# bluenote-1577/floria

Measured on AMD Instinct MI355X. Metric: SNP-blocks phased/sec (whole node), higher is better.
Workload: dtype u64 (Q24 fixed-point allele weights) + f64 scores

## Files before the change

### floria_amd/csrc/floria_hip.hip

```cpp
#include <hip/hip_runtime.h>

#include <algorithm>
#include <cmath>
#include <cstdint>
#include <cstdio>
#include <cstdlib>
#include <cstring>
#include <limits>
#include <numeric>
#include <string>
#include <utility>
#include <atomic>
#include <chrono>
#include <mutex>
#include <thread>
#include <type_traits>
#include <vector>

#include "../../include/floria_hip.h"
#include "beam_kernel.h"
#include "wave_util.h"
#include "beam_slab_kernel.h"
#include "beam_wide_kernel.h"
#include "optimize_kernel.h"
#include "reassign_kernel.h"
#include "hapq_kernel.h"
#include "blocks_kernel.h"
#include "graph_kernel.h"
#include "stats_kernel.h"
#include "realign_kernel.h"
#include "realign_walk_kernel.h"
#include "pileup_kernel.h"
#include "realign_gather_kernel.h"
#include "upload_kernel.h"
#include "assemble_kernel.h"
#include "assemble_order_kernel.h"
#include "mono_kernel.h"
#include "span_kernel.h"

static_assert(FLORIA_MAX_PLOIDY == fl::MAX_PLOIDY, "ploidy limits out of sync");

namespace {

thread_local std::string g_err;
int fail(int code, const std::string& msg) { g_err = msg; return code; }

#define HIPCHK(expr)                                                                                   \
    do {                                                                                               \
        hipError_t _e = (expr);                                                                        \
        if (_e != hipSuccess)                                                                          \
            return fail(_e == hipErrorOutOfMemory ? FLORIA_E_NOMEM : FLORIA_E_DEVICE,                  \
                        std::string(#expr) + ": " + hipGetErrorString(_e));                            \
    } while (0)

constexpr double DIV_FACTOR  = 0.25;
constexpr double PROB_CUTOFF = 0.01;
constexpr uint32_t BINOM_NMAX_CAP = 1024;

struct DevBuf {
    void* p = nullptr;
    size_t cap = 0;
    int ensure(size_t bytes) {
        if (bytes <= cap) return 0;
        if (p) { (void)hipFree(p); p = nullptr; cap = 0; }
        size_t want = bytes + bytes / 8 + 256;
        hipError_t e = hipMalloc(&p, want);
        if (e != hipSuccess) { p = nullptr; return fail(FLORIA_E_NOMEM, std::string("hipMalloc(") + std::to_string(want) + "): " + hipGetErrorString(e)); }
        cap = want;
        return 0;
    }
    void release() { if (p) (void)hipFree(p); p = nullptr; cap = 0; }
    template <class T> T* as() const { return (T*)p; }
};

struct Seg { size_t off, bytes; };
struct Carve {
    size_t cursor = 0;
    char* base = nullptr;
    Seg seg(size_t bytes) { const Seg s{cursor, bytes}; cursor += (bytes + 255) & ~(size_t)255; return s; }
    int place(DevBuf& buf) { const int rc = buf.ensure(cursor + 256); base = buf.as<char>(); return rc; }
    template <class T = void> T* at(Seg s) const { return (T*)(base + s.off); }
    hipError_t up(Seg s, const void* src, size_t bytes, hipStream_t st) const { return bytes ? hipMemcpyAsync(base + s.off, src, bytes, hipMemcpyHostToDevice, st) : hipSuccess; }
};

struct HostBox {
    char* h = nullptr;
    char* d = nullptr;
    size_t cap = 0;
    int ensure(size_t bytes) {
        if (bytes <= cap) return 0;
        release();
        const size_t want = bytes + bytes / 4 + 4096;
        hipError_t e = hipHostMalloc((void**)&h, want, hipHostMallocMapped);
        if (e == hipSuccess) e = hipHostGetDevicePointer((void**)&d, h, 0);
        if (e != hipSuccess) { if (h) (void)hipHostFree(h); h = nullptr; d = nullptr; return fail(FLORIA_E_NOMEM, std::string("hipHostMalloc(mapped, ") + std::to_string(want) + "): " + hipGetErrorString(e)); }
        cap = want;
        return 0;
    }
    void release() { if (h) (void)hipHostFree(h); h = nullptr; d = nullptr; cap = 0; }
};

struct StagePool {
    static constexpr size_t SEG = 16u << 20;
    static constexpr uint32_t NBUF = 8;
    char* buf[NBUF] = {};
    hipEvent_t ev[NBUF] = {};
    bool used[NBUF] = {};
    int init() {
        for (uint32_t i = 0; i < NBUF; ++i) if (!buf[i]) {
            if (hipHostMalloc((void**)&buf[i], SEG, hipHostMallocDefault) != hipSuccess) return fail(FLORIA_E_NOMEM, "hipHostMalloc(staging) failed");
            if (hipEventCreateWithFlags(&ev[i], hipEventDisableTiming) != hipSuccess) return fail(FLORIA_E_DEVICE, "hipEventCreate failed");
        }
        return 0;
    }
    void release() { for (uint32_t i = 0; i < NBUF; ++i) { if (buf[i]) (void)hipHostFree(buf[i]); if (ev[i]) (void)hipEventDestroy(ev[i]); buf[i] = nullptr; ev[i] = nullptr; used[i] = false; } }
};

uint64_t splitmix64(uint64_t& s) {
    uint64_t z = (s += 0x9e3779b97f4a7c15ull);
    z = (z ^ (z >> 30)) * 0xbf58476d1ce4e5b9ull;
    z = (z ^ (z >> 27)) * 0x94d049bb133111ebull;
    return z ^ (z >> 31);
}

}

namespace {
struct BigCache {
    std::mutex m;
    std::vector<std::pair<void*, size_t>> v;
    void* get(size_t n) {
        {
            std::lock_guard<std::mutex> l(m);
            for (size_t i = 0; i < v.size(); ++i)
                if (v[i].second >= n && v[i].second <= 2 * n + 4096) { void* b = v[i].first; v.erase(v.begin() + i); return (char*)b + 64; }
        }
        void* b = malloc(n + 64);
        if (!b) return nullptr;
        *(size_t*)b = n;
        return (char*)b + 64;
    }
    void put(void* payload) {
        if (!payload) return;
        void* b = (char*)payload - 64;
        const size_t cap = *(size_t*)b;
        std::lock_guard<std::mutex> l(m);
        if (cap >= (1u << 20) && v.size() < 8) v.push_back({b, cap}); else free(b);
    }
};
BigCache g_big;
}

struct Knobs {
    uint32_t groups = 0;
    uint32_t beam_path = 0;
    uint32_t no_specialized = 0;
    uint32_t no_p1_shortcut = 0;
    uint32_t opt_threads = 0;
    uint32_t opt_global = 0;
    int32_t  speculate = -1;
    uint32_t upload_chunks = 0;
    uint32_t trace = 0;
    uint32_t spec_gate_div = 2;
    uint32_t reassign_path = 0;
    uint32_t no_bulk = 0;
    uint32_t fx_tags = 0;
    uint32_t arith_ow6 = 0;
    uint32_t asm_order_general = 0;
    uint32_t chain_wgs = 0;
    uint32_t arith_replay = 0;
    uint32_t arith_hbm = 0;
    uint32_t opt_block_order = 0;
    uint32_t s2_assign_only = 0;
    uint32_t arith = 0;
    int32_t  tail_overlap = 0;
    uint32_t tail_waves = 2;
};

struct Arena;

struct floria_hip_ctx {
    int device = 0;
    uint32_t hw_queues = 0;
    hipStream_t stream = nullptr;
    uint32_t user_slots = 0;
    Knobs knobs;
    int n_cu = 256;
    static constexpr uint32_t MAX_GROUPS = 8;
    static constexpr uint32_t MAX_LANES = 32;
    hipStream_t gstream[MAX_LANES] = {};
    hipStream_t gstream_low[MAX_LANES] = {};
    hipEvent_t ev_fork[MAX_LANES] = {}, ev_join[MAX_LANES] = {};
    hipEvent_t ev_gate[MAX_GROUPS] = {};
    hipStream_t tstream[MAX_GROUPS] = {};
    hipEvent_t ev_tail[MAX_GROUPS] = {}, ev_tail_join[MAX_GROUPS] = {};
    hipStream_t copy_stream = nullptr;
    hipEvent_t ev_rids = nullptr;
    hipEvent_t ev_chunk[MAX_GROUPS + 1] = {};
    hipEvent_t ev_copied[MAX_GROUPS + 1] = {};
    hipStream_t flat_stream = nullptr;
    HostBox box;
    double binom_eps = -1.0;
    uint32_t binom_nmax = 0;
    DevBuf d_binom;
    DevBuf d_hash;
    uint32_t hash_len = 0;
    uint32_t w24[256];
    DevBuf d_w24;
    uint64_t Rk1[FLORIA_MAX_PLOIDY], Rk2[FLORIA_MAX_PLOIDY];
    DevBuf state_pool, hist_pool, opt_hist, opt_dist, opt_gain, opt_key, opt_moves, misc, misc0;
    uint32_t cur_len_max = 0;
    uint64_t upload_epoch = 0, ord_epoch = ~0ull, ord_sig = 0;
    const uint2* cur_ord = nullptr; const uint64_t* cur_ord_off = nullptr;
    DevBuf arith_ord, arith_scr, arith_tab, arith_pool;
    floria_timing timing{};
    uint64_t batch_token = 0, token_counter = 0;
    fl::BlockSet last_bs{};
    const uint8_t* last_part = nullptr;
    const uint32_t* last_best = nullptr;
    uint32_t last_nall = 2;
    std::vector<uint32_t> last_bc, last_start, last_end;
    DevBuf graph_buf, graph_hist, graph_sort;
    DevBuf up_tmp;
    std::vector<Arena*> arena_cache;
    StagePool stage;
    DevBuf pile_in, pile_out;
    uint64_t res_token = 0;
    const floria_record_summary* res_summary = nullptr;
    uint32_t res_n_contigs = 0;
    std::vector<uint32_t> res_contig;
    const uint64_t* res_cell_off = nullptr; const uint32_t* res_snp = nullptr; const uint8_t *res_allele = nullptr, *res_qual = nullptr;
    const uint32_t* res_seq_pos = nullptr;
    DevBuf asm_plan;
// ... 1410 lines not shown
                          if (P > 3) { stages.emplace_back(); for (uint32_t p = 4; p <= P; ++p) stages.back().push_back(p); } }
    else for (uint32_t p = 1; p <= P; ++p) stages.push_back({p});
    if (spec == 3 && P < 5) { stages.clear(); for (uint32_t p = 1; p <= P; ++p) stages.push_back({p}); }
    return stages;
}

int s1_core(floria_hip_ctx* ctx, const S1Contigs& SC, const uint32_t* blk_contig, const uint32_t* blk_start, const uint32_t* blk_end,
            uint32_t n_blocks, const floria_params* prm, floria_block_result** out) {
    const uint32_t n_contigs = (uint32_t)SC.cdev.size();
    const Trace TR(ctx->knobs.trace);
    TR.mark("s1_core enter");
    if (prm->max_ploidy < 1 || prm->max_ploidy > FLORIA_MAX_PLOIDY) return fail(FLORIA_E_INVALID, "max_ploidy must be in 1..16");
    if (prm->beam < 1) return fail(FLORIA_E_INVALID, "beam (max_number_solns) must be >= 1");
    if (!(prm->epsilon > 0.0 && prm->epsilon < 1.0)) return fail(FLORIA_E_INVALID, "epsilon must be in (0,1)");
    ctx->timing = floria_timing{};
    ctx->batch_token = 0;
    const uint32_t P = prm->max_ploidy;

    std::vector<uint32_t> bc(n_blocks, 0);
    uint32_t n_max = 1, span_max = 1;
    const uint32_t len_max = SC.len_max, nall = SC.nall;
    const bool any_q0 = SC.any_q0;
    for (uint32_t b = 0; b < n_blocks; ++b) {
        const uint32_t ci = blk_contig ? blk_contig[b] : 0;
        if (ci >= n_contigs) return fail(FLORIA_E_INVALID, "blk_contig out of range");
        bc[b] = ci;
    }
    const std::vector<fl::ContigDev>& cdev = SC.cdev;
    Carve C0;
    const Seg s_cdev = C0.seg(sizeof(fl::ContigDev) * std::max(1u, n_contigs)), s_bc = C0.seg(4ull * n_blocks + 4), s_bs = C0.seg(4ull * n_blocks + 4),
              s_be = C0.seg(4ull * n_blocks + 4), s_p0 = C0.seg(4ull * n_blocks + 4), s_sp = C0.seg(4ull * n_blocks + 4), s_cnt = C0.seg(4ull * n_blocks + 4),
              s_bytes = C0.seg(8ull * n_blocks + 8), s_roff = C0.seg(8ull * (n_blocks + 1));
    int rc = C0.place(ctx->misc0); if (rc) return rc;
    EventTimer T(ctx->stream);
    static_assert(sizeof(fl::ContigDev) % 4 == 0, "box_copy_kernel moves 4-byte words");
    size_t box_cur = 0;
    auto box_take = [&](size_t bytes) { const size_t o = box_cur; box_cur += (bytes + 63) & ~(size_t)63; return o; };
    const size_t bx_cdev = box_take(sizeof(fl::ContigDev) * n_contigs), bx_bc = box_take(4ull * n_blocks), bx_bs = box_take(4ull * n_blocks), bx_be = box_take(4ull * n_blocks),
                 bx_cnt = box_take(4ull * n_blocks), bx_span = box_take(4ull * n_blocks), bx_bytes = box_take(8ull * n_blocks), bx_roff = box_take(8ull * (n_blocks + 1)),
                 bx_jobs = box_take(4ull * n_blocks);
    rc = ctx->box.ensure(box_cur + 64); if (rc) return rc;
    auto box_up = [&](void* dst, const void* src, size_t bytes, size_t at) -> hipError_t {
        if (!bytes) return hipSuccess;
        memcpy(ctx->box.h + at, src, bytes);
        const uint32_t words = (uint32_t)(bytes / 4);
        hipLaunchKernelGGL(box_copy_kernel, dim3(std::max(1u, std::min(256u, (words + 255) / 256))), dim3(256), 0, ctx->stream, (uint32_t*)dst, (const uint32_t*)(ctx->box.d + at), words);
        return hipGetLastError();
    };
    int th = T.begin(K_H2D);
    HIPCHK(box_up(C0.at(s_cdev), cdev.data(), sizeof(fl::ContigDev) * n_contigs, bx_cdev));
    if (n_blocks) {
        HIPCHK(box_up(C0.at(s_bc), bc.data(), 4ull * n_blocks, bx_bc));
        HIPCHK(box_up(C0.at(s_bs), blk_start, 4ull * n_blocks, bx_bs));
        HIPCHK(box_up(C0.at(s_be), blk_end, 4ull * n_blocks, bx_be));
    }
    T.end(th);
    fl::ScanArgs sa{};
    sa.contigs = C0.at<const fl::ContigDev>(s_cdev);
    sa.blk_contig = C0.at<const uint32_t>(s_bc); sa.blk_start = C0.at<const uint32_t>(s_bs); sa.blk_end = C0.at<const uint32_t>(s_be);
    sa.n_blocks = n_blocks; sa.max_ploidy = P;
    sa.cnt = C0.at<uint32_t>(s_cnt); sa.pos0 = C0.at<uint32_t>(s_p0); sa.span = C0.at<uint32_t>(s_sp); sa.bytes = C0.at<uint64_t>(s_bytes);
    sa.h_cnt = (uint32_t*)(ctx->box.d + bx_cnt); sa.h_span = (uint32_t*)(ctx->box.d + bx_span); sa.h_bytes = (uint64_t*)(ctx->box.d + bx_bytes);
    std::vector<uint32_t> cnt(n_blocks, 0), span(n_blocks, 0);
    std::vector<uint64_t> blk_bytes(n_blocks, 0), roff(n_blocks + 1, 0);
    if (n_blocks) {
        int tk = T.begin(K_SEL);
        hipLaunchKernelGGL(fl::block_reads_kernel<false>, dim3(n_blocks), dim3(64), 0, ctx->stream, sa);
        T.end(tk);
        HIPCHK(hipGetLastError());
        HIPCHK(hipStreamSynchronize(ctx->stream));
        memcpy(cnt.data(), ctx->box.h + bx_cnt, 4ull * n_blocks);
        memcpy(span.data(), ctx->box.h + bx_span, 4ull * n_blocks);
        memcpy(blk_bytes.data(), ctx->box.h + bx_bytes, 8ull * n_blocks);
    }
    TR.mark("block counts on the host");
    uint64_t algo_bytes = 0;
    for (uint32_t b = 0; b < n_blocks; ++b) {
        roff[b + 1] = roff[b] + cnt[b];
        n_max = std::max(n_max, cnt[b]); span_max = std::max(span_max, span[b]);
        algo_bytes += blk_bytes[b];
    }
    if (n_max >= (1u << 20)) return fail(FLORIA_E_UNSUPPORTED, "more than 2^20 reads in one block");
    const uint64_t tot = roff[n_blocks];
    std::vector<uint32_t> jobs;
    for (uint32_t b = 0; b < n_blocks; ++b) if (cnt[b]) jobs.push_back(b);
    std::stable_sort(jobs.begin(), jobs.end(), [&](uint32_t a, uint32_t b2) { return cnt[a] > cnt[b2]; });
    TR.mark("jobs sorted");
    const bool chunked = SC.chunk_ev != nullptr && SC.n_chunks > 1;
    hipEvent_t group_ev[floria_hip_ctx::MAX_GROUPS] = {};
    const std::vector<uint32_t> group_off = job_groups(ctx, SC, chunked, bc, jobs, group_ev);
    const std::vector<std::vector<uint32_t>> stages = ploidy_stages(ctx, prm, jobs.size(), (uint32_t)group_off.size() - 1);
    uint32_t stage_w = 1;
    for (auto& st : stages) stage_w = std::max<uint32_t>(stage_w, (uint32_t)st.size());

    rc = ensure_binom(ctx, prm->epsilon, len_max); if (rc) return rc;
    if (span_max > fl::HASH_M) return fail(FLORIA_E_UNSUPPORTED, "a block's reads span more than 65536 SNPs");
    rc = ensure_hash(ctx, span_max * nall); if (rc) return rc;

    Carve C;
    const Seg s_rids = C.seg(4ull * tot + 4), s_jobs = C.seg(4ull * jobs.size() + 4), s_planes = C.seg((uint64_t)P * tot + 16), s_bpart = C.seg((uint64_t)(stage_w + 1) * (tot + 16)),
              s_margin = C.seg(8ull * n_blocks * P + 16),
              s_out = C.seg(tot + 16), s_mec = C.seg(8ull * n_blocks * P + 8), s_na = C.seg(8ull * n_blocks * P + 8), s_it = C.seg(4ull * n_blocks * P + 4),
              s_done = C.seg(n_blocks + 4), s_best = C.seg(4ull * n_blocks + 4), s_tried = C.seg(4ull * n_blocks + 4), s_ready = C.seg(4ull * n_blocks + 4),
              s_q = C.seg(8ull * floria_hip_ctx::MAX_LANES * FLORIA_MAX_PLOIDY + 16), s_diag = C.seg(16 + 8 * 64), s_steps = C.seg(16);
    const size_t zero_bytes = C.cursor - s_out.off;
    const Seg s_stop = C.seg(4ull * n_blocks + 4);
    rc = C.place(ctx->misc); if (rc) return rc;
    th = T.begin(K_H2D);
    HIPCHK(box_up(C0.at(s_roff), roff.data(), 8ull * (n_blocks + 1), bx_roff));
    if (!jobs.empty()) HIPCHK(box_up(C.at(s_jobs), jobs.data(), 4ull * jobs.size(), bx_jobs));
    HIPCHK(hipMemsetAsync(C.at(s_out), 0, zero_bytes, ctx->stream));
    if (stage_w > 1) HIPCHK(hipMemsetAsync(C.at(s_stop), 0xff, s_stop.bytes, ctx->stream));
    const double inf = std::numeric_limits<double>::infinity();
    T.end(th);
    if (n_blocks) {
        sa.roff = C0.at<const uint64_t>(s_roff); sa.rids = C.at<uint32_t>(s_rids);
        int tk = T.begin(K_SEL);
        hipLaunchKernelGGL(fl::block_reads_kernel<true>, dim3(n_blocks), dim3(64), 0, ctx->stream, sa);
        T.end(tk);
        HIPCHK(hipGetLastError());
        if (!ctx->ev_rids) HIPCHK(hipEventCreateWithFlags(&ctx->ev_rids, hipEventDisableTiming));
        if (!ctx->copy_stream) HIPCHK(hipStreamCreateWithFlags(&ctx->copy_stream, hipStreamNonBlocking));
        HIPCHK(hipEventRecord(ctx->ev_rids, ctx->stream));
    }

    fl::BlockSet bs{};
    bs.contigs = C0.at<const fl::ContigDev>(s_cdev);
    bs.blk_contig = C0.at<const uint32_t>(s_bc); bs.blk_start = C0.at<const uint32_t>(s_bs); bs.blk_end = C0.at<const uint32_t>(s_be);
    bs.blk_pos0 = C0.at<const uint32_t>(s_p0); bs.blk_span = C0.at<const uint32_t>(s_sp);
    bs.blk_read_off = C0.at<const uint64_t>(s_roff); bs.blk_read = C.at<const uint32_t>(s_rids); bs.n_blocks = n_blocks;

    ctx->cur_ord = nullptr; ctx->cur_ord_off = nullptr; ctx->cur_len_max = len_max;
    if (ctx->knobs.arith && n_contigs && SC.orders_in_flight) {
        ctx->cur_ord = ctx->arith_ord.as<uint2>(); ctx->cur_ord_off = ctx->arith_tab.as<uint64_t>() + n_contigs + 1;
    } else if (ctx->knobs.arith && n_contigs) {
        if (SC.n_cells.size() != n_contigs || chunked) return fail(FLORIA_E_INVALID, "internal: the reference-arithmetic mode needs resident contigs");
        int tk = T.begin(K_SEL);
        rc = cell_orders(ctx, bs.contigs, cdev, SC.n_cells, len_max);
        T.end(tk);
        if (rc) return rc;
    }

    floria_block_result* R = (floria_block_result*)calloc(1, sizeof(floria_block_result));
    if (!R) return fail(FLORIA_E_NOMEM, "calloc");
    R->n_blocks = n_blocks; R->max_ploidy = P;
    R->best_ploidy = (uint32_t*)calloc(n_blocks + 1, 4);
    R->ploidies_tried = (uint32_t*)calloc(n_blocks + 1, 4);
    R->read_off = (uint64_t*)calloc(n_blocks + 1, 8);
    R->read_id = (uint32_t*)g_big.get(4 * (tot + 1));
    R->part = (uint8_t*)g_big.get(tot + 1);
    R->mec = (double*)calloc((size_t)n_blocks * P + 1, 8);
    struct ResultGuard { floria_hip_ctx* c; floria_block_result* r; ~ResultGuard() { if (r) { sync_all(c); floria_hip_block_result_free(r); } } } guard{ctx, R};
    if (!R->best_ploidy || !R->ploidies_tried || !R->read_off || !R->read_id || !R->part || !R->mec) { return fail(FLORIA_E_NOMEM, "malloc"); }
    bool p1_shortcut = false;
    const PhaseShape shape{bs, any_q0, (uint32_t)jobs.size(), tot, n_max, span_max};
    const PhaseBufs bufs{C.at<const uint32_t>(s_jobs), C.at<uint8_t>(s_planes), C.at<uint8_t>(s_bpart), C.at<double>(s_mec), C.at<double>(s_na), C.at<uint32_t>(s_it),
                         C.at<uint8_t>(s_done), C.at<uint32_t>(s_best), C.at<uint32_t>(s_tried), C.at<uint32_t>(s_stop), C.at<uint32_t>(s_ready), C.at<uint32_t>(s_q),
                         C.at<double>(s_margin), C.at<uint32_t>(s_diag), C.at<unsigned long long>(s_steps)};
    auto run = nall == 2 ? run_phase<2> : run_phase<4>;
    rc = run(ctx, prm, shape, group_off, stages, chunked ? group_ev : nullptr, bufs, T, p1_shortcut);
    if (rc) { sync_all(ctx); return rc; }
    TR.mark("every launch queued");
    int t_rids = -1;
    if (n_blocks && tot) {
        HIPCHK(hipStreamWaitEvent(ctx->copy_stream, ctx->ev_rids, 0));
        t_rids = T.begin(K_D2H, ctx->copy_stream);
        hipError_t ce = hipMemcpyAsync(R->read_id, C.at(s_rids), 4ull * tot, hipMemcpyDeviceToHost, ctx->copy_stream);
        T.end(t_rids);
        if (ce != hipSuccess) { sync_all(ctx); return fail(FLORIA_E_DEVICE, hipGetErrorString(ce)); }
    }
    {
        int t = T.begin(K_SEL);
        if (n_blocks) hipLaunchKernelGGL(fl::gather_kernel, dim3(n_blocks), dim3(64), 0, ctx->stream, n_blocks, bs.blk_read_off,
                                         C.at<const uint32_t>(s_best), C.at<const uint8_t>(s_planes), tot, C.at<uint8_t>(s_out));
        T.end(t);
        HIPCHK(hipGetLastError());
    }

    int td = T.begin(K_D2H);
    hipError_t e = hipSuccess;
    uint32_t diag[4] = {0, 0, 0, 0};
    unsigned long long steps = 0;
    double margin = inf;
    if (n_blocks) {
        e = hipMemcpyAsync(R->best_ploidy, C.at(s_best), 4ull * n_blocks, hipMemcpyDeviceToHost, ctx->stream);
        if (e == hipSuccess) e = hipMemcpyAsync(R->ploidies_tried, C.at(s_tried), 4ull * n_blocks, hipMemcpyDeviceToHost, ctx->stream);
        if (e == hipSuccess) e = hipMemcpyAsync(R->mec, C.at(s_mec), 8ull * n_blocks * P, hipMemcpyDeviceToHost, ctx->stream);
        if (e == hipSuccess && tot) e = hipMemcpyAsync(R->part, C.at(s_out), tot, hipMemcpyDeviceToHost, ctx->stream);
    }
    if (e == hipSuccess) e = hipMemcpyAsync(diag, C.at(s_diag), 16, hipMemcpyDeviceToHost, ctx->stream);
    if (e == hipSuccess) e = hipMemcpyAsync(&steps, C.at(s_steps), 8, hipMemcpyDeviceToHost, ctx->stream);
    std::vector<double> job_margin((size_t)n_blocks * P + 1, inf);
    if (e == hipSuccess && n_blocks) e = hipMemcpyAsync(job_margin.data(), C.at(s_margin), 8ull * n_blocks * P, hipMemcpyDeviceToHost, ctx->stream);
    T.end(td);
    if (e == hipSuccess) e = hipStreamSynchronize(ctx->stream);
    if (e == hipSuccess && ctx->copy_stream) e = hipStreamSynchronize(ctx->copy_stream);
    if (e != hipSuccess) { sync_all(ctx); return fail(FLORIA_E_DEVICE, std::string("phase_blocks: ") + hipGetErrorString(e)); }
    TR.mark("results on the host");
    if (diag[1]) { return fail(FLORIA_E_DEVICE, "internal: beam slab free-list underflow"); }
#ifdef FLORIA_PROF
    { unsigned long long prof[64]; (void)hipMemcpy(prof, C.at<char>(s_diag) + 16, sizeof(prof), hipMemcpyDeviceToHost); fprintf(stderr, "[prof]"); for (int i = 0; i < 64; ++i) fprintf(stderr, " %d:%.1fM", i, prof[i] / 1e6); fprintf(stderr, "\n"); }
#endif
    memcpy(R->read_off, roff.data(), 8ull * (n_blocks + 1));
    for (uint32_t b = 0; b < n_blocks; ++b)
        for (uint32_t p = (p1_shortcut ? 2 : 1); p <= R->ploidies_tried[b]; ++p) margin = std::min(margin, job_margin[(size_t)b * P + p - 1]);
    if (p1_shortcut && !jobs.empty()) margin = std::min(margin, std::fabs(0.0 - std::log(PROB_CUTOFF)));
    R->min_prune_margin = margin;
    ctx->timing.beam_ms = T.sum(K_BEAM); ctx->timing.optimize_ms = T.sum(K_OPT); ctx->timing.select_ms = T.sum(K_SEL);
    ctx->timing.beam_union_ms = T.union_ms(K_BEAM); ctx->timing.optimize_union_ms = T.union_ms(K_OPT);
    ctx->timing.h2d_ms = T.sum(K_H2D); ctx->timing.d2h_ms = T.sum(K_D2H); ctx->timing.total_ms = T.span(); ctx->timing.phase_ms = T.sum(K_PHASE);
    ctx->timing.algorithmic_bytes = algo_bytes; ctx->timing.beam_steps = steps;
    std::vector<uint32_t> stage_first(P + 2, 0);
    for (auto& st : stages) for (uint32_t p : st) stage_first[p] = st.front();
    for (uint32_t b = 0; b < n_blocks; ++b) {
        const uint32_t tb = R->ploidies_tried[b];
        uint32_t launches_b = 0;
        for (uint32_t p = 1; p <= P && tb; ++p) if (tb >= stage_first[p] && !(p == 1 && p1_shortcut)) launches_b++;
        ctx->timing.beam_launch_bytes += blk_bytes[b] * launches_b; ctx->timing.jobs += tb;
    }
    ctx->batch_token = R->batch_token = ++ctx->token_counter;
    ctx->last_bs = bs; ctx->last_part = C.at<const uint8_t>(s_out); ctx->last_best = C.at<const uint32_t>(s_best); ctx->last_nall = nall;
    ctx->last_bc = bc; ctx->last_start.assign(blk_start, blk_start + n_blocks); ctx->last_end.assign(blk_end, blk_end + n_blocks);
    guard.r = nullptr;
    *out = R;
    return 0;
}

}

extern "C" {

int floria_hip_phase_blocks_batch(floria_hip_ctx* ctx, const floria_hip_contig* const* contigs, uint32_t n_contigs,
                                  const uint32_t* blk_contig, const uint32_t* blk_start, const uint32_t* blk_end,
                                  uint32_t n_blocks, const floria_params* prm, floria_block_result** out) {
    if (!ctx || !out || !prm || (n_blocks && (!blk_start || !blk_end || !contigs))) return fail(FLORIA_E_INVALID, "null argument");
    *out = nullptr;
    HIPCHK(hipSetDevice(ctx->device));
    S1Contigs SC;
    SC.cdev.resize(n_contigs);
    SC.n_cells.assign(n_contigs, 0);
    for (uint32_t b = 0; b < n_blocks; ++b) {
        const uint32_t ci = blk_contig ? blk_contig[b] : 0;
        if (ci >= n_contigs || !contigs[ci]) return fail(FLORIA_E_INVALID, "blk_contig out of range");
    }
    for (uint32_t i = 0; i < n_contigs; ++i) if (contigs[i]) {
        if (contigs[i]->ctx != ctx) return fail(FLORIA_E_INVALID, "contig belongs to another context");
        SC.cdev[i] = contigs[i]->dev;
        SC.n_cells[i] = contigs[i]->n_cells;
        SC.len_max = std::max(SC.len_max, contigs[i]->max_len);
        SC.nall = std::max(SC.nall, contigs[i]->n_alleles);
        SC.any_q0 = SC.any_q0 || contigs[i]->has_q0;
    }
    return s1_core(ctx, SC, blk_contig, blk_start, blk_end, n_blocks, prm, out);
}

static int phase_pileups_impl(floria_hip_ctx* ctx, const floria_pileup* pileups, const floria_pileup_packed* pk, uint32_t n_contigs,
                              const uint32_t* blk_contig, const uint32_t* blk_start, const uint32_t* blk_end, uint32_t n_blocks,
                              const floria_params* prm, floria_block_result** out, floria_hip_contig** keep) {
    if (!ctx || !out || !prm || (n_contigs && !pileups && !pk) || (n_blocks && (!blk_start || !blk_end))) return fail(FLORIA_E_INVALID, "null argument");
    *out = nullptr;
    if (keep) for (uint32_t i = 0; i < n_contigs; ++i) keep[i] = nullptr;
    HIPCHK(hipSetDevice(ctx->device));
    for (uint32_t b = 0; b < n_blocks; ++b) if ((blk_contig ? blk_contig[b] : 0) >= n_contigs) return fail(FLORIA_E_INVALID, "blk_contig out of range");
    if (n_contigs == 0) { S1Contigs SC; return s1_core(ctx, SC, blk_contig, blk_start, blk_end, n_blocks, prm, out); }
    uint64_t cells = 0;
    auto n_reads_of = [&](uint32_t i) { return pk ? pk[i].n_reads : pileups[i].n_reads; };
    for (uint32_t i = 0; i < n_contigs; ++i) { const uint32_t* ro = pk ? pk[i].read_off : pileups[i].read_off; if (n_reads_of(i) && ro) cells += ro[n_reads_of(i)]; }
    uint32_t want_chunks = ctx->knobs.upload_chunks ? ctx->knobs.upload_chunks : (uint32_t)std::max<uint64_t>(cells * 6 >= (160ull << 20) ? 2 : 1, std::min<uint64_t>(5, cells * 6 / (200ull << 20)));
    if (ctx->knobs.arith && !ctx->knobs.upload_chunks) want_chunks = std::min<uint32_t>(want_chunks, 2);
    UploadPlan UP;
    uint32_t chunk_cap = floria_hip_ctx::MAX_GROUPS;
    if (!ctx->knobs.upload_chunks && ctx->knobs.speculate < 0 && prm->max_ploidy >= 3) {
        if (n_blocks <= (uint32_t)ctx->n_cu * 18) chunk_cap = std::max<uint32_t>(1, 10 / prm->max_ploidy);
        else if (n_blocks <= (uint32_t)ctx->n_cu * 23 && prm->max_ploidy >= 4) chunk_cap = std::max<uint32_t>(1, 10 / std::max<uint32_t>(3, prm->max_ploidy - 3));
    }
    int rc = plan_upload(ctx, pileups, pk, n_contigs, std::min<uint32_t>(std::min(want_chunks, chunk_cap), floria_hip_ctx::MAX_GROUPS), UP);
    if (rc) return rc;
    std::vector<floria_hip_contig*> handles(n_contigs, nullptr);
    auto drop = [&](int code) { sync_all(ctx); for (auto* h : handles) if (h) { h->arena = nullptr; delete h; } arena_put(UP.A); return code; };
    bool pipelined = UP.all_pinned && UP.n_chunks > 1;
    const bool arith_pipe = pipelined && ctx->knobs.arith != 0;
    OrderPlan OP;
    std::vector<fl::ContigDev> pipe_cdev;
    std::vector<uint64_t> pipe_cells;
    const uint64_t order_scratch = 64ull << 20;
    uint64_t pinned_b = 0, staged_b = 0;
    floria_block_result* R = nullptr;
    if (pipelined) {
        if (!ctx->copy_stream) HIPCHK(hipStreamCreateWithFlags(&ctx->copy_stream, hipStreamNonBlocking));
        if (!ctx->flat_stream) {
            int lo = 0, hi = 0;
            (void)hipDeviceGetStreamPriorityRange(&lo, &hi);
            if (hipStreamCreateWithPriority(&ctx->flat_stream, hipStreamNonBlocking, hi) != hipSuccess) { (void)hipGetLastError(); HIPCHK(hipStreamCreateWithFlags(&ctx->flat_stream, hipStreamNonBlocking)); }
        }
// ... 36 lines not shown
                const int orc = order_launch(ctx, OP, (const fl::ContigDev*)(ctx->arith_tab.as<char>() + ord_cdev_off), c0, c1, ctx->arith_scr.as<uint64_t>() + OP.pre[c0] + g,
                                             ctx->arith_scr.as<uint8_t>() + ((8 * ord_todo_words + 255) & ~(size_t)255), order_scratch, 0,
                                             &((const fl::UploadStatus*)(UP.T + UP.t_st) + c0)->max_len, ctx->flat_stream);
                if (orc) rc = orc;
            }
            if (e == hipSuccess) e = hipEventRecord(ctx->ev_chunk[g], ctx->flat_stream);
        }
        if (!rc && e != hipSuccess) rc = fail(FLORIA_E_DEVICE, std::string("pipelined upload: ") + hipGetErrorString(e));
        if (rc) return drop(rc);
        S1Contigs SC;
        SC.cdev = pipe_cdev;
        if (arith_pipe) { SC.n_cells = pipe_cells; SC.orders_in_flight = true; }
        SC.len_max = BINOM_NMAX_CAP; SC.nall = 2; SC.any_q0 = false;
        SC.contig_chunk = UP.contig_chunk.data(); SC.n_chunks = UP.n_chunks; SC.chunk_ev = ctx->ev_chunk;
        if (pk) { SC.chunk_groups = 3; SC.ends_apart = true; }
        rc = s1_core(ctx, SC, blk_contig, blk_start, blk_end, n_blocks, prm, &R);
        if (rc) return drop(rc);
        const floria_timing tm = ctx->timing;
        hipError_t e2 = hipMemcpy(UP.ust.data(), UP.T + UP.t_st, sizeof(fl::UploadStatus) * n_contigs, hipMemcpyDeviceToHost);
        if (e2 != hipSuccess) { floria_hip_block_result_free(R); return drop(fail(FLORIA_E_DEVICE, std::string("upload status: ") + hipGetErrorString(e2))); }
        rc = finish_upload(ctx, UP, handles.data());
        if (!rc && arith_pipe) {
            uint64_t bad = 0;
            e2 = hipMemcpy(&bad, ctx->arith_tab.as<uint64_t>() + 2 * (size_t)n_contigs + 2, 8, hipMemcpyDeviceToHost);
            if (e2 != hipSuccess) rc = fail(FLORIA_E_DEVICE, std::string("set-order status: ") + hipGetErrorString(e2));
            else rc = order_bad_read(OP, bad);
            if (!rc) { ctx->ord_epoch = ctx->upload_epoch; ctx->ord_sig = OP.sig; }
            if (rc) { floria_hip_block_result_free(R); for (auto* h : handles) floria_hip_contig_free(h); return rc; }
        }
        if (rc) { floria_hip_block_result_free(R); for (auto*& h : handles) h = nullptr; return drop(rc); }
        bool plan_ok = true;
        for (auto* h : handles) plan_ok = plan_ok && h->n_alleles == 2 && !h->has_q0;
        if (!plan_ok) {
            floria_hip_block_result_free(R); R = nullptr;
            rc = floria_hip_phase_blocks_batch(ctx, handles.data(), n_contigs, blk_contig, blk_start, blk_end, n_blocks, prm, &R);
            if (rc) { for (auto* h : handles) floria_hip_contig_free(h); return rc; }
        } else ctx->timing = tm;
    } else {
        arena_put(UP.A);
        rc = upload_batch_impl(ctx, pileups, pk, n_contigs, handles.data());
        if (rc) return rc;
        pinned_b = ctx->timing.upload_pinned_bytes; staged_b = ctx->timing.upload_staged_bytes;
        rc = floria_hip_phase_blocks_batch(ctx, handles.data(), n_contigs, blk_contig, blk_start, blk_end, n_blocks, prm, &R);
        if (rc) { for (auto* h : handles) floria_hip_contig_free(h); return rc; }
    }
    ctx->timing.upload_pinned_bytes = pinned_b; ctx->timing.upload_staged_bytes = staged_b; ctx->timing.upload_chunks = pipelined ? UP.n_chunks : 1;
    if (keep) for (uint32_t i = 0; i < n_contigs; ++i) keep[i] = handles[i];
    else { for (auto* h : handles) floria_hip_contig_free(h); ctx->batch_token = 0; R->batch_token = 0; }
    *out = R;
    return 0;
}

int floria_hip_phase_pileups_batch(floria_hip_ctx* ctx, const floria_pileup* pileups, uint32_t n_contigs,
                                   const uint32_t* blk_contig, const uint32_t* blk_start, const uint32_t* blk_end, uint32_t n_blocks,
                                   const floria_params* prm, floria_block_result** out, floria_hip_contig** keep) {
    return phase_pileups_impl(ctx, pileups, nullptr, n_contigs, blk_contig, blk_start, blk_end, n_blocks, prm, out, keep);
}
int floria_hip_phase_pileups_batch_packed(floria_hip_ctx* ctx, const floria_pileup_packed* pileups, uint32_t n_contigs,
                                          const uint32_t* blk_contig, const uint32_t* blk_start, const uint32_t* blk_end, uint32_t n_blocks,
                                          const floria_params* prm, floria_block_result** out, floria_hip_contig** keep) {
    return phase_pileups_impl(ctx, nullptr, pileups, n_contigs, blk_contig, blk_start, blk_end, n_blocks, prm, out, keep);
}

int floria_hip_phase_blocks_resident(floria_hip_ctx* ctx, const floria_hip_contig* contig, const uint32_t* blk_start,
                                     const uint32_t* blk_end, uint32_t n_blocks, const floria_params* params,
                                     floria_block_result** out) {
    if (!contig) return fail(FLORIA_E_INVALID, "null contig");
    const floria_hip_contig* arr[1] = {contig};
    return floria_hip_phase_blocks_batch(ctx, arr, 1, nullptr, blk_start, blk_end, n_blocks, params, out);
}

int floria_hip_phase_blocks(floria_hip_ctx* ctx, const floria_pileup* pileup, const uint32_t* blk_start, const uint32_t* blk_end,
                            uint32_t n_blocks, const floria_params* params, floria_block_result** out) {
    floria_hip_contig* c = nullptr;
    int rc = floria_hip_contig_upload(ctx, pileup, &c);
    if (rc) return rc;
    rc = floria_hip_phase_blocks_resident(ctx, c, blk_start, blk_end, n_blocks, params, out);
    floria_hip_contig_free(c);
    return rc;
}

void floria_hip_block_result_free(floria_block_result* r) {
    if (!r) return;
    free(r->best_ploidy); free(r->ploidies_tried); free(r->read_off); g_big.put(r->read_id); g_big.put(r->part); free(r->mec); free(r);
}

int floria_hip_hap_graph(floria_hip_ctx* ctx, const floria_block_result* res, floria_hap_graph** out) {
    if (!ctx || !res || !out) return fail(FLORIA_E_INVALID, "null argument");
    *out = nullptr;
    if (!ctx->batch_token || res->batch_token != ctx->batch_token) return fail(FLORIA_E_INVALID, "the batch is no longer resident: call floria_hip_hap_graph directly after phase_blocks");
    HIPCHK(hipSetDevice(ctx->device));
    const uint32_t nb = res->n_blocks;
    floria_hap_graph* G = (floria_hap_graph*)calloc(1, sizeof(floria_hap_graph));
    if (!G) return fail(FLORIA_E_NOMEM, "calloc");
    G->n_blocks = nb;
    G->node_off = (uint64_t*)calloc(nb + 1, 8); G->edge_off = (uint64_t*)calloc(nb + 1, 8); G->pred = (int32_t*)calloc(nb + 1, 4);
    uint32_t range_max = 1, pmax = 1;
    {
        std::vector<int32_t> last_of_contig;
        for (uint32_t b = 0; b < nb; ++b) {
            const uint32_t ci = ctx->last_bc[b];
            if (ci >= last_of_contig.size()) last_of_contig.resize(ci + 1, -1);
            const uint32_t p2 = res->best_ploidy[b];
            G->pred[b] = -1;
            G->node_off[b + 1] = G->node_off[b] + p2;
            G->edge_off[b + 1] = G->edge_off[b];
            if (p2) {
                G->pred[b] = last_of_contig[ci];
                if (G->pred[b] >= 0) G->edge_off[b + 1] += (uint64_t)res->best_ploidy[G->pred[b]] * p2;
                last_of_contig[ci] = (int32_t)b;
                range_max = std::max(range_max, ctx->last_end[b] - ctx->last_start[b] + 1);
                pmax = std::max(pmax, p2);
            }
        }
    }
    const uint64_t n_nodes = G->node_off[nb], n_edges = G->edge_off[nb];
    G->node_cov = (double*)calloc(n_nodes + 1, 8); G->edge_w = (uint32_t*)calloc(n_edges + 1, 4);
    if (!G->node_off || !G->edge_off || !G->pred || !G->node_cov || !G->edge_w) { floria_hip_hap_graph_free(G); return fail(FLORIA_E_NOMEM, "calloc"); }
    if (nb == 0) { *out = G; return 0; }
    const uint32_t A = ctx->last_nall;
    Carve C;
    const Seg s_pred = C.seg(4ull * nb), s_noff = C.seg(8ull * (nb + 1)), s_eoff = C.seg(8ull * (nb + 1)), s_cov = C.seg(8ull * n_nodes + 8), s_ew = C.seg(4ull * n_edges + 4);
    int rc = C.place(ctx->graph_buf);
    const size_t hist_bytes = (size_t)range_max * pmax * A * 8;
    const bool in_lds = hist_bytes <= 40 * 1024;
    uint64_t sort_cap = 1;
    while (sort_cap < (uint64_t)range_max * A) sort_cap <<= 1;
    if (!rc && !in_lds) rc = ctx->graph_hist.ensure((uint64_t)nb * hist_bytes);
    if (!rc && (uint64_t)range_max * A > (uint64_t)fl::GRAPH_SORT_CAP) rc = ctx->graph_sort.ensure((uint64_t)nb * sort_cap * 8);
    if (rc) { floria_hip_hap_graph_free(G); return rc; }
    hipError_t e = C.up(s_pred, G->pred, 4ull * nb, ctx->stream);
    if (e == hipSuccess) e = C.up(s_noff, G->node_off, 8ull * (nb + 1), ctx->stream);
    if (e == hipSuccess) e = C.up(s_eoff, G->edge_off, 8ull * (nb + 1), ctx->stream);
    fl::GraphArgs a{};
    a.bs = ctx->last_bs; a.best_ploidy = ctx->last_best; a.part = ctx->last_part;
    a.pred = C.at<const int32_t>(s_pred); a.node_off = C.at<const uint64_t>(s_noff); a.edge_off = C.at<const uint64_t>(s_eoff);
    a.node_cov = C.at<double>(s_cov); a.edge_w = C.at<uint32_t>(s_ew);
    a.hist_pool = ctx->graph_hist.as<uint64_t>(); a.sort_pool = ctx->graph_sort.as<uint64_t>(); a.sort_cap = sort_cap;
    a.range_max = range_max; a.hist_in_lds = in_lds ? 1 : 0; a.hist_stride = hist_bytes / 8;
    EventTimer T(ctx->stream);
    int tk = T.begin(K_SEL);
    if (e == hipSuccess) {
        if (A == 2) hipLaunchKernelGGL(fl::graph_kernel<2>, dim3(nb), dim3(fl::GRAPH_THREADS), in_lds ? hist_bytes : 0, ctx->stream, a);
        else hipLaunchKernelGGL(fl::graph_kernel<4>, dim3(nb), dim3(fl::GRAPH_THREADS), in_lds ? hist_bytes : 0, ctx->stream, a);
        e = hipGetLastError();
    }
    T.end(tk);
    if (e == hipSuccess && n_nodes) e = hipMemcpyAsync(G->node_cov, C.at(s_cov), 8ull * n_nodes, hipMemcpyDeviceToHost, ctx->stream);
    if (e == hipSuccess && n_edges) e = hipMemcpyAsync(G->edge_w, C.at(s_ew), 4ull * n_edges, hipMemcpyDeviceToHost, ctx->stream);
    if (e == hipSuccess) e = hipStreamSynchronize(ctx->stream);
    if (e != hipSuccess) { floria_hip_hap_graph_free(G); return fail(FLORIA_E_DEVICE, std::string("hap_graph: ") + hipGetErrorString(e)); }
    ctx->timing.select_ms = T.sum(K_SEL);
    *out = G;
    return 0;
}
void floria_hip_hap_graph_free(floria_hap_graph* g) {
    if (!g) return;
    free(g->node_off); free(g->node_cov); free(g->pred); free(g->edge_off); free(g->edge_w); free(g);
}

int floria_hip_haploset_stats(floria_hip_ctx* ctx, const floria_hip_contig* const* contigs, uint32_t n_contigs,
                              const uint32_t* grp_contig, const uint64_t* grp_off, const uint32_t* grp_read,
                              const uint32_t* grp_range, uint32_t n_groups, double* out4) {
    if (!ctx || (n_contigs && !contigs) || (n_groups && (!grp_off || !grp_range || !out4))) return fail(FLORIA_E_INVALID, "null argument");
    if (n_groups == 0) return 0;
    HIPCHK(hipSetDevice(ctx->device));
    ctx->batch_token = 0;
// ... 1225 lines not shown
```

Measured before the change: 185,300.

## Use pinned host result buffers, coalesce small D2H copies, counting-sort jobs

Result arrays for partitions and read ids now come from a cache of pinned host buffers, so device-to-host copies can run as true DMA instead of being staged through pageable memory. The device misc segments are reordered so best ploidy, tried ploidies, MEC, margins, steps and diagnostics sit contiguously and come back in one copy instead of six. The job ordering replaces the stable comparison sort with a counting sort by read count. The risks are the cost of pinned allocation on cache misses and more complex ownership of the carved result memory.

```diff
diff --git a/floria_amd/csrc/floria_hip.hip b/floria_amd/csrc/floria_hip.hip
--- a/floria_amd/csrc/floria_hip.hip
+++ b/floria_amd/csrc/floria_hip.hip
@@ -37,6 +37,7 @@
 #include "assemble_order_kernel.h"
 #include "mono_kernel.h"
 #include "span_kernel.h"
+#include "job_order.h"
 
 static_assert(FLORIA_MAX_PLOIDY == fl::MAX_PLOIDY, "ploidy limits out of sync");
 
@@ -149,6 +150,37 @@
     }
 };
 BigCache g_big;
+
+struct PinnedCache {
+    std::mutex m;
+    std::vector<std::pair<void*, size_t>> v;
+    static void release(void* b) { if (((size_t*)b)[1]) (void)hipHostFree(b); else free(b); }
+    void* get(size_t n) {
+        {
+            std::lock_guard<std::mutex> l(m);
+            for (size_t i = 0; i < v.size(); ++i)
+                if (v[i].second >= n && v[i].second <= 2 * n + 4096) { void* b = v[i].first; v.erase(v.begin() + i); return (char*)b + 64; }
+        }
+        void* b = nullptr;
+        size_t pinned = 1;
+        if (hipHostMalloc(&b, n + 64, hipHostMallocPortable) != hipSuccess || !b) { (void)hipGetLastError(); b = malloc(n + 64); pinned = 0; }
+        if (!b) return nullptr;
+        ((size_t*)b)[0] = n; ((size_t*)b)[1] = pinned;
+        return (char*)b + 64;
+    }
+    void put(void* payload) {
+        if (!payload) return;
+        void* b = (char*)payload - 64;
+        void* old = nullptr;
+        {
+            std::lock_guard<std::mutex> l(m);
+            if (v.size() >= 8) { old = v.front().first; v.erase(v.begin()); }
+            v.push_back({b, *(size_t*)b});
+        }
+        if (old) release(old);
+    }
+};
+PinnedCache g_pinned;
 }
 
 struct Knobs {
@@ -1725,9 +1757,7 @@
     }
     if (n_max >= (1u << 20)) return fail(FLORIA_E_UNSUPPORTED, "more than 2^20 reads in one block");
     const uint64_t tot = roff[n_blocks];
-    std::vector<uint32_t> jobs;
-    for (uint32_t b = 0; b < n_blocks; ++b) if (cnt[b]) jobs.push_back(b);
-    std::stable_sort(jobs.begin(), jobs.end(), [&](uint32_t a, uint32_t b2) { return cnt[a] > cnt[b2]; });
+    std::vector<uint32_t> jobs = fl::lpt_order(cnt.data(), n_blocks);
     TR.mark("jobs sorted");
     const bool chunked = SC.chunk_ev != nullptr && SC.n_chunks > 1;
     hipEvent_t group_ev[floria_hip_ctx::MAX_GROUPS] = {};
@@ -1742,17 +1772,19 @@
 
     Carve C;
     const Seg s_rids = C.seg(4ull * tot + 4), s_jobs = C.seg(4ull * jobs.size() + 4), s_planes = C.seg((uint64_t)P * tot + 16), s_bpart = C.seg((uint64_t)(stage_w + 1) * (tot + 16)),
-              s_margin = C.seg(8ull * n_blocks * P + 16),
-              s_out = C.seg(tot + 16), s_mec = C.seg(8ull * n_blocks * P + 8), s_na = C.seg(8ull * n_blocks * P + 8), s_it = C.seg(4ull * n_blocks * P + 4),
-              s_done = C.seg(n_blocks + 4), s_best = C.seg(4ull * n_blocks + 4), s_tried = C.seg(4ull * n_blocks + 4), s_ready = C.seg(4ull * n_blocks + 4),
-              s_q = C.seg(8ull * floria_hip_ctx::MAX_LANES * FLORIA_MAX_PLOIDY + 16), s_diag = C.seg(16 + 8 * 64), s_steps = C.seg(16);
-    const size_t zero_bytes = C.cursor - s_out.off;
+              s_best = C.seg(4ull * n_blocks + 4), s_tried = C.seg(4ull * n_blocks + 4), s_mec = C.seg(8ull * n_blocks * P + 8), s_margin = C.seg(8ull * n_blocks * P + 16),
+              s_steps = C.seg(16), s_diag = C.seg(16 + 8 * 64),
+              s_out = C.seg(tot + 16), s_na = C.seg(8ull * n_blocks * P + 8), s_it = C.seg(4ull * n_blocks * P + 4),
+              s_done = C.seg(n_blocks + 4), s_ready = C.seg(4ull * n_blocks + 4),
+              s_q = C.seg(8ull * floria_hip_ctx::MAX_LANES * FLORIA_MAX_PLOIDY + 16);
+    const size_t zero_bytes = C.cursor - s_best.off;
+    const size_t small_bytes = s_diag.off + 16 - s_best.off;
     const Seg s_stop = C.seg(4ull * n_blocks + 4);
     rc = C.place(ctx->misc); if (rc) return rc;
     th = T.begin(K_H2D);
     HIPCHK(box_up(C0.at(s_roff), roff.data(), 8ull * (n_blocks + 1), bx_roff));
     if (!jobs.empty()) HIPCHK(box_up(C.at(s_jobs), jobs.data(), 4ull * jobs.size(), bx_jobs));
-    HIPCHK(hipMemsetAsync(C.at(s_out), 0, zero_bytes, ctx->stream));
+    HIPCHK(hipMemsetAsync(C.at(s_best), 0, zero_bytes, ctx->stream));
     if (stage_w > 1) HIPCHK(hipMemsetAsync(C.at(s_stop), 0xff, s_stop.bytes, ctx->stream));
     const double inf = std::numeric_limits<double>::infinity();
     T.end(th);
@@ -1787,14 +1819,20 @@
     floria_block_result* R = (floria_block_result*)calloc(1, sizeof(floria_block_result));
     if (!R) return fail(FLORIA_E_NOMEM, "calloc");
     R->n_blocks = n_blocks; R->max_ploidy = P;
-    R->best_ploidy = (uint32_t*)calloc(n_blocks + 1, 4);
-    R->ploidies_tried = (uint32_t*)calloc(n_blocks + 1, 4);
+    char* const small = (char*)g_pinned.get(small_bytes);
     R->read_off = (uint64_t*)calloc(n_blocks + 1, 8);
-    R->read_id = (uint32_t*)g_big.get(4 * (tot + 1));
-    R->part = (uint8_t*)g_big.get(tot + 1);
-    R->mec = (double*)calloc((size_t)n_blocks * P + 1, 8);
+    R->read_id = (uint32_t*)g_pinned.get(4 * (tot + 1));
+    R->part = (uint8_t*)g_pinned.get(tot + 1);
+    if (small) {
+        R->best_ploidy = (uint32_t*)small;
+        R->ploidies_tried = (uint32_t*)(small + (s_tried.off - s_best.off));
+        R->mec = (double*)(small + (s_mec.off - s_best.off));
+    }
     struct ResultGuard { floria_hip_ctx* c; floria_block_result* r; ~ResultGuard() { if (r) { sync_all(c); floria_hip_block_result_free(r); } } } guard{ctx, R};
-    if (!R->best_ploidy || !R->ploidies_tried || !R->read_off || !R->read_id || !R->part || !R->mec) { return fail(FLORIA_E_NOMEM, "malloc"); }
+    if (!small || !R->read_off || !R->read_id || !R->part) { return fail(FLORIA_E_NOMEM, "malloc"); }
+    const double* const job_margin = (const double*)(small + (s_margin.off - s_best.off));
+    const uint32_t* const diag = (const uint32_t*)(small + (s_diag.off - s_best.off));
+    const unsigned long long* const steps = (const unsigned long long*)(small + (s_steps.off - s_best.off));
     bool p1_shortcut = false;
     const PhaseShape shape{bs, any_q0, (uint32_t)jobs.size(), tot, n_max, span_max};
     const PhaseBufs bufs{C.at<const uint32_t>(s_jobs), C.at<uint8_t>(s_planes), C.at<uint8_t>(s_bpart), C.at<double>(s_mec), C.at<double>(s_na), C.at<uint32_t>(s_it),
@@ -1821,20 +1859,9 @@
     }
 
     int td = T.begin(K_D2H);
-    hipError_t e = hipSuccess;
-    uint32_t diag[4] = {0, 0, 0, 0};
-    unsigned long long steps = 0;
     double margin = inf;
-    if (n_blocks) {
-        e = hipMemcpyAsync(R->best_ploidy, C.at(s_best), 4ull * n_blocks, hipMemcpyDeviceToHost, ctx->stream);
-        if (e == hipSuccess) e = hipMemcpyAsync(R->ploidies_tried, C.at(s_tried), 4ull * n_blocks, hipMemcpyDeviceToHost, ctx->stream);
-        if (e == hipSuccess) e = hipMemcpyAsync(R->mec, C.at(s_mec), 8ull * n_blocks * P, hipMemcpyDeviceToHost, ctx->stream);
-        if (e == hipSuccess && tot) e = hipMemcpyAsync(R->part, C.at(s_out), tot, hipMemcpyDeviceToHost, ctx->stream);
-    }
-    if (e == hipSuccess) e = hipMemcpyAsync(diag, C.at(s_diag), 16, hipMemcpyDeviceToHost, ctx->stream);
-    if (e == hipSuccess) e = hipMemcpyAsync(&steps, C.at(s_steps), 8, hipMemcpyDeviceToHost, ctx->stream);
-    std::vector<double> job_margin((size_t)n_blocks * P + 1, inf);
-    if (e == hipSuccess && n_blocks) e = hipMemcpyAsync(job_margin.data(), C.at(s_margin), 8ull * n_blocks * P, hipMemcpyDeviceToHost, ctx->stream);
+    hipError_t e = n_blocks && tot ? hipMemcpyAsync(R->part, C.at(s_out), tot, hipMemcpyDeviceToHost, ctx->stream) : hipSuccess;
+    if (e == hipSuccess) e = hipMemcpyAsync(small, C.at(s_best), small_bytes, hipMemcpyDeviceToHost, ctx->stream);
     T.end(td);
     if (e == hipSuccess) e = hipStreamSynchronize(ctx->stream);
     if (e == hipSuccess && ctx->copy_stream) e = hipStreamSynchronize(ctx->copy_stream);
@@ -1852,7 +1879,7 @@
     ctx->timing.beam_ms = T.sum(K_BEAM); ctx->timing.optimize_ms = T.sum(K_OPT); ctx->timing.select_ms = T.sum(K_SEL);
     ctx->timing.beam_union_ms = T.union_ms(K_BEAM); ctx->timing.optimize_union_ms = T.union_ms(K_OPT);
     ctx->timing.h2d_ms = T.sum(K_H2D); ctx->timing.d2h_ms = T.sum(K_D2H); ctx->timing.total_ms = T.span(); ctx->timing.phase_ms = T.sum(K_PHASE);
-    ctx->timing.algorithmic_bytes = algo_bytes; ctx->timing.beam_steps = steps;
+    ctx->timing.algorithmic_bytes = algo_bytes; ctx->timing.beam_steps = *steps;
     std::vector<uint32_t> stage_first(P + 2, 0);
     for (auto& st : stages) for (uint32_t p : st) stage_first[p] = st.front();
     for (uint32_t b = 0; b < n_blocks; ++b) {
@@ -2055,7 +2082,7 @@
 
 void floria_hip_block_result_free(floria_block_result* r) {
     if (!r) return;
-    free(r->best_ploidy); free(r->ploidies_tried); free(r->read_off); g_big.put(r->read_id); g_big.put(r->part); free(r->mec); free(r);
+    g_pinned.put(r->best_ploidy); free(r->read_off); g_pinned.put(r->read_id); g_pinned.put(r->part); free(r);
 }
 
 int floria_hip_hap_graph(floria_hip_ctx* ctx, const floria_block_result* res, floria_hap_graph** out) {
diff --git a/floria_amd/csrc/job_order.h b/floria_amd/csrc/job_order.h
--- /dev/null
+++ b/floria_amd/csrc/job_order.h
@@ -0,0 +1,28 @@
+#pragma once
+#include <algorithm>
+#include <cstdint>
+#include <vector>
+
+namespace fl {
+
+inline std::vector<uint32_t> lpt_order(const uint32_t* cnt, uint32_t n) {
+    std::vector<uint32_t> jobs;
+    uint32_t top = 0, live = 0;
+    for (uint32_t b = 0; b < n; ++b) { top = std::max(top, cnt[b]); live += cnt[b] != 0; }
+    if (!live) return jobs;
+    if (top >= (1u << 20)) {
+        jobs.reserve(live);
+        for (uint32_t b = 0; b < n; ++b) if (cnt[b]) jobs.push_back(b);
+        std::stable_sort(jobs.begin(), jobs.end(), [&](uint32_t a, uint32_t b2) { return cnt[a] > cnt[b2]; });
+        return jobs;
+    }
+    std::vector<uint32_t> at((size_t)top + 2, 0);
+    for (uint32_t b = 0; b < n; ++b) at[cnt[b]]++;
+    uint32_t run = 0;
+    for (uint32_t c = top; c >= 1; --c) { const uint32_t h = at[c]; at[c] = run; run += h; }
+    jobs.resize(live);
+    for (uint32_t b = 0; b < n; ++b) if (cnt[b]) jobs[at[cnt[b]]++] = b;
+    return jobs;
+}
+
+}
```

Result: no change. 187,100, median of 6 (+0.9%).
